# hohMiyazawa/hoh-ANS

Measured on NVIDIA B200. Metric: raw RGB MB/s, encode+decode (BASELINE.json: raw RGB MB/s encode & decode, % of HBM peak), higher is better.
Workload: dtype u8/u16 pixels, u32 freqs, u64 rANS state (integer)

## Files before the change

### hoh-ans_b200/csrc/hoh_api.cu

```cuda
#include <cuda_runtime.h>

#include <algorithm>
#include <cmath>
#include <cstdio>
#include <cstdlib>
#include <cstring>
#include <map>
#include <string>
#include <vector>

#include "hoh_kernels.cuh"

using namespace hohk;

namespace {

enum Slot {
    S_FREQS = 0, S_CUM, S_HEADS, S_ENCMETA, S_DECMETA, S_RESID, S_STREAMS, S_DSTREAMS, S_DRESULTS,
    S_IO_A, S_IO_B, S_IO_C, S_IO_D, S_IO_E, S_RESULTS, S_TOP, S_BP, S_HIST, S_COST, S_SUMS, S_MASKS,
    S_WIDE_TOP, S_WIDE_BP, S_MISC, S_L_MAPS, S_L_IDX, S_L_HDR, S_L_U32, S_L_STATUS, S_L_RR, S_L_RES, S_LZ_PX, S_LZ_STATE, S_LZ_SIDE, S_LZ_COUNTS, S_LZ_SLABS, S_LZ_RES, S_LZ_BONUS, S_LZ_KEYS, S_LZ_VALS, S_LZ_FLAG, S_T_NUKE, S_T_LZ, S_T_U32, S_T_P8, S_T_P9, S_T_O8, S_T_O9, S_T_R8, S_T_R9, S_T_MORE_SHAPES, S_T_LAST = S_T_NUKE + 4 * 9 - 1, S_D_TILES, S_D_PLANES, S_D_LZSYM, S_D_IDXSYM, S_D_RESID, S_D_OUT, S_D_BACKREF, S_D_MAPS,
    S_D_STREAMS, S_D_RES_A, S_D_RES_B, S_D_TOP, S_D_BP, S_D_PSTATUS, S_L_NEED, S_L_ORDER, S_COUNT
};

struct Buf {
// ... 772 lines not shown
    if (stream_len == 0 || stream_len % 8 || slab_bytes % 16) return HOH_E_ARG;
    if (n == 0) return HOH_OK;
    const uint64_t streams = (n + stream_len - 1) / stream_len;
    const unsigned sgrid = blocks_for(streams, kStaticWarps * 32);
    if (prob_bits >= 14) {
        k_rans_encode_static<0><<<sgrid, kStaticWarps * 32, 0, ctx->stream>>>(d_symbols, n, stream_len, d_cum, range, prob_bits, d_out,
                                                                          slab_bytes, d_payload_bytes);
    } else {
        k_rans_encode_static<1><<<sgrid, kStaticWarps * 32, 0, ctx->stream>>>(d_symbols, n, stream_len, d_cum, range, prob_bits, d_out,
                                                                          slab_bytes, d_payload_bytes);
    }
    LAUNCHED("k_rans_encode_static");
    return HOH_OK;
}

int hoh_rans_decode_static(hoh_ctx* ctx, const uint8_t* d_in, uint32_t slab_bytes,
                           const uint32_t* d_payload_bytes, size_t n, uint32_t stream_len,
                           const uint32_t* d_cum, uint32_t range, uint32_t prob_bits, uint16_t* d_symbols) {
    DeviceGuard guard_(ctx);
    if (!ctx || !d_symbols || !d_cum || !d_in || !d_payload_bytes) return HOH_E_ARG;
    if (range == 0 || range > HOH_MAX_RANGE || prob_bits == 0 || prob_bits > HOH_MAX_PROB_BITS) return HOH_E_UNSUPPORTED;
    if (stream_len == 0 || stream_len % 8 || slab_bytes % 16) return HOH_E_ARG;
    if (n == 0) return HOH_OK;
    const uint64_t streams = (n + stream_len - 1) / stream_len;
    if (prob_bits <= 15) {
        const size_t sym_bytes = range <= 256 ? 1 : 2;
        const size_t smem = (size_t)kStaticDirectWarps * 32 * kRingWords * 4 + (size_t)kStaticDirectWarps * 32 * kDecStride * 2 +
                            (size_t)HOH_MAX_RANGE * 4 + ((size_t)sym_bytes << prob_bits);
        TRY(ensure_smem_opt_in(ctx));
        const unsigned blocks = blocks_for(streams, kStaticDirectWarps * 32);
        if (range <= 256)
            k_rans_decode_static_direct<uint8_t><<<blocks, kStaticDirectWarps * 32, smem, ctx->stream>>>(
                d_in, slab_bytes, d_payload_bytes, n, stream_len, d_cum, range, prob_bits, d_symbols);
        else
            k_rans_decode_static_direct<uint16_t><<<blocks, kStaticDirectWarps * 32, smem, ctx->stream>>>(
                d_in, slab_bytes, d_payload_bytes, n, stream_len, d_cum, range, prob_bits, d_symbols);
        LAUNCHED("k_rans_decode_static_direct");
        return HOH_OK;
    }
    k_rans_decode_static<<<blocks_for(streams, kStaticDecWarps * 32), kStaticDecWarps * 32, 0, ctx->stream>>>(
        d_in, slab_bytes, d_payload_bytes, n, stream_len, d_cum, range, prob_bits, d_symbols);
    LAUNCHED("k_rans_decode_static");
    return HOH_OK;
}

int hoh_tile_geometry_for(uint32_t width, uint32_t height, hoh_tile_geometry* out) {
    if (!out || width == 0 || height == 0) return HOH_E_ARG;
    hoh_tile_geometry g;
    g.width = width;
    g.height = height;
    if ((width >= 512 || height >= 512) && width >= 256 && height >= 256) {
        g.x_tiles = width / 256;
        g.y_tiles = height / 256;
    } else {
        g.x_tiles = g.y_tiles = 1;
    }
    g.tile_w = (width + g.x_tiles - 1) / g.x_tiles;
    g.tile_h = (height + g.y_tiles - 1) / g.y_tiles;
    g.tiles_per_image = g.x_tiles * g.y_tiles;
    g.streams_per_image = 3 * g.tiles_per_image;
    *out = g;
    return HOH_OK;
}

size_t hoh_encode_images_out_bytes(const hoh_tile_geometry* g, size_t n_images) {
    if (!g) return 0;
    return hoh_enc_slab_bytes((size_t)g->tile_w * g->tile_h, 15) * g->streams_per_image * n_images;
}

int hoh_encode_images_s0(hoh_ctx* ctx, const uint8_t* d_rgb, size_t n_images, uint32_t width, uint32_t height,
                         const uint8_t* d_nuke, uint8_t* d_out, size_t out_bytes, hoh_stream_result* d_results,
                         uint8_t* d_packed, size_t packed_cap, uint64_t* d_packed_off) {
    DeviceGuard guard_(ctx);
    if (!ctx || !d_rgb || !d_out || !d_results) return HOH_E_ARG;
    if (n_images == 0) return HOH_OK;
    hoh_tile_geometry hg;
    TRY(hoh_tile_geometry_for(width, height, &hg));
    if ((uint64_t)hg.tile_w * hg.tile_h >= (1u << 21)) return HOH_E_UNSUPPORTED;
    const TileGeom g = to_geom(hg);
    const uint64_t n_tiles = (uint64_t)n_images * g.tiles_per_image, n_streams = n_tiles * 3;
    const uint32_t slab = (uint32_t)hoh_enc_slab_bytes((size_t)g.tile_w * g.tile_h, 15);
    if (out_bytes < n_streams * slab) return HOH_E_CAPACITY;
    uint16_t* resid;
    uint32_t* freqs;
    hoh_enc_stream* streams;
    TRY(scratch_t(ctx, S_RESID, n_streams * g.plane_stride, &resid));
    TRY(scratch_t(ctx, S_FREQS, n_streams * kFreqRow, &freqs));
    TRY(scratch_t(ctx, S_STREAMS, n_streams, &streams));
    if (g.width % 4 == 0 && g.tile_w % 4 == 0 && g.tile_w <= 1024) {
        k_tile_residuals_s0<<<(unsigned)n_tiles, 256, 0, ctx->stream>>>(d_rgb, g, resid, freqs);
    } else {
        k_tile_residuals_s0_generic<<<(unsigned)n_tiles, 256, 0, ctx->stream>>>(d_rgb, g, resid, freqs);
    }
    LAUNCHED("k_tile_residuals_s0");
    k_make_tile_streams<<<blocks_for(n_streams, 256), 256, 0, ctx->stream>>>(g, n_tiles, slab, streams);
    LAUNCHED("k_make_tile_streams");
    if (d_nuke) {
        k_compact_nuke<<<blocks_for(n_streams * 32, 128), 128, 0, ctx->stream>>>(g, n_tiles, d_nuke, g.plane_stride, resid,
                                                                                streams);
        LAUNCHED("k_compact_nuke");
        k_histogram<<<(unsigned)n_streams, 256, 0, ctx->stream>>>(streams, resid, freqs);
        LAUNCHED("k_histogram");
    }
    TRY(encode_from_freqs(ctx, streams, n_streams, resid, d_out, d_results, freqs, 512, 15, 15, true));
    if (d_packed) {
        if (!d_packed_off) return HOH_E_ARG;
        k_scan_sizes<<<1, 1024, 0, ctx->stream>>>(d_results, (uint32_t)n_streams, d_packed_off);
        LAUNCHED("k_scan_sizes");
        k_gather_streams<<<(unsigned)n_streams, 256, 0, ctx->stream>>>(d_results, d_out, d_packed_off, d_packed,
                                                                       packed_cap);
        LAUNCHED("k_gather_streams");
    }
    return HOH_OK;
}


int hoh_decode_images_s0(hoh_ctx* ctx, const uint8_t* d_packed, size_t packed_bytes, const uint64_t* d_packed_off,
                         size_t n_images, uint32_t width, uint32_t height, const uint16_t* d_backref,
                         uint8_t* d_rgb, int32_t* d_status) {
    DeviceGuard guard_(ctx);
    if (!ctx || !d_packed || !d_packed_off || !d_rgb || !d_status) return HOH_E_ARG;
    if (n_images == 0) return HOH_OK;
    if (packed_bytes < 32) return HOH_E_ARG;
    hoh_tile_geometry hg;
    TRY(hoh_tile_geometry_for(width, height, &hg));
    const TileGeom g = to_geom(hg);
    const uint64_t n_tiles = (uint64_t)n_images * g.tiles_per_image, n_streams = n_tiles * 3;
    uint16_t* resid;
    hoh_dec_stream* streams;
    hoh_dec_result* results;
    TRY(scratch_t(ctx, S_DSTREAMS, n_streams, &streams));
    TRY(scratch_t(ctx, S_DRESULTS, n_streams, &results));
    const bool fused = !d_backref && g.tile_w * g.x_tiles == g.width && g.tile_h * g.y_tiles == g.height && g.tile_w % 8 == 0 &&
                       g.tile_w >= 16 && g.width % 8 == 0 && (reinterpret_cast<uintptr_t>(d_rgb) & 7u) == 0 &&
                       !getenv("HOH_NO_FUSED_DECODE");
    if (fused) {
        uint32_t* cum;
        DecMeta* meta;
        TRY(scratch_t(ctx, S_CUM, n_streams * kCumRow, &cum));
        TRY(scratch_t(ctx, S_DECMETA, n_streams, &meta));
        TRY(ensure_smem_opt_in(ctx));
        k_make_tile_dec_streams<<<blocks_for(n_streams, 256), 256, 0, ctx->stream>>>(g, n_tiles, d_packed, packed_bytes,
                                                                                     d_packed_off, streams, d_status);
        LAUNCHED("k_make_tile_dec_streams");
        k_parse_streams<<<blocks_for(n_streams, kTableWarps), kTableWarps * 32, 0, ctx->stream>>>(
            streams, (uint32_t)n_streams, d_packed, packed_bytes, cum, meta, results);
        LAUNCHED("k_parse_streams");
        const uint32_t classes[5] = {0, 64, 128, 256, HOH_MAX_RANGE + 3};
        const bool overlap = !ctx->profiling;
        if (overlap) TRY(aux_fork(ctx, 4));
        const unsigned grid = blocks_for(n_tiles, kFusedTiles);
        for (int c = 0; c < 4; c++) {
            const uint32_t rows = classes[c + 1];
            const size_t fixed = (size_t)rows * 32 * sizeof(uint32_t) + 32 * kRingWords * sizeof(uint32_t) + kFusedStage;
            const size_t lut_bytes = (size_t)kLutSize * 32 * (rows <= 256 ? 1 : 2);
            const size_t smem = smem_even_share(ctx, fixed + lut_bytes, grid);
            cudaStream_t sc = overlap ? ctx->aux[c] : ctx->stream;
            if (rows <= 256) {
                k_rans_decode_tiles_s0<uint8_t><<<grid, 32, smem, sc>>>(
                    streams, (uint32_t)n_streams, d_packed, packed_bytes, cum, meta, results, g, d_rgb, d_status, classes[c], rows);
            } else {
                k_rans_decode_tiles_s0<uint16_t><<<grid, 32, smem, sc>>>(
                    streams, (uint32_t)n_streams, d_packed, packed_bytes, cum, meta, results, g, d_rgb, d_status, classes[c], rows);
            }
            static const char* const names[4] = {"k_rans_decode_tiles_s0[rows<=64]", "k_rans_decode_tiles_s0[rows<=128]",
                                                 "k_rans_decode_tiles_s0[rows<=256]", "k_rans_decode_tiles_s0[rows<=515]"};
            LAUNCHED(names[c]);
        }
        if (overlap) TRY(aux_join(ctx, 4));
        return HOH_OK;
    }
    TRY(scratch_t(ctx, S_RESID, n_streams * g.plane_stride, &resid));
    const size_t unp_smem = (size_t)kUnpWarps * ((32 * kRingStride + g.tile_w + (g.tile_w + 1) / 2 + 3) & ~(size_t)3) * sizeof(uint32_t);
    if (unp_smem > 200 * 1024) return HOH_E_UNSUPPORTED;
    k_make_tile_dec_streams<<<blocks_for(n_streams, 256), 256, 0, ctx->stream>>>(g, n_tiles, d_packed, packed_bytes,
                                                                                 d_packed_off, streams, d_status);
    LAUNCHED("k_make_tile_dec_streams");
    TRY(decode_common(ctx, streams, n_streams, d_packed, packed_bytes, resid, results));
    k_merge_status<<<blocks_for(n_streams, 256), 256, 0, ctx->stream>>>(results, n_streams, g, d_backref ? 0u : 1u, d_status);
    LAUNCHED("k_merge_status");
    if (d_backref) {
        uint16_t* planes;
        TRY(scratch_t(ctx, S_D_OUT, n_streams * g.plane_stride, &planes));
        k_tile_unpredict_s0_backref<<<blocks_for(n_streams, 64), 64, 0, ctx->stream>>>(resid, g, n_tiles, results, d_backref,
                                                                                      planes, d_status);
        LAUNCHED("k_tile_unpredict_s0_backref");
        k_tile_store_s0<<<(unsigned)n_tiles, 256, 0, ctx->stream>>>(planes, g, d_rgb);
// ... 1306 lines not shown
```

### hoh-ans_b200/csrc/hoh_kernels.cuh

```cuda
#pragma once
#include <cuda_runtime.h>
#include <stdint.h>

#include <type_traits>

#include "../../include/hohgpu.h"
#include "hoh_format.cuh"

namespace hohk {

constexpr int kFreqRow = 512;
constexpr int kCumRow = 520;
constexpr int kChunk = 64;
static_assert(true, "");
constexpr int kGroup = 8;
constexpr int kSymStride = 66;
constexpr uint64_t kRansL = 1ull << 31;
constexpr int kDecChunk = 32;
constexpr int kDecStride = 34;
constexpr uint32_t kSymBits = 9;
constexpr uint32_t kSymMask = (1u << kSymBits) - 1u;

struct EncMeta {
    uint64_t payload_start;
// ... 320 lines not shown
    }
    if (!__all_sync(0xffffffffu, fits)) {
        uint32_t len = 0;
        if (lane == 0) len = hohfmt::build_head(f, range, n, prob_bits, buf, stored_size);
        len = __shfl_sync(0xffffffffu, len, 0);
        *stored_size = __shfl_sync(0xffffffffu, *stored_size, 0);
        __syncwarp();
        return len;
    }
    const uint32_t pair_bits = mode == 2u ? 2u * count * maxbits : 0u;
    uint32_t bit = warp_incl_scan(my_bits) - my_bits + 8u * at + pair_bits;
    const uint32_t total_bits = __shfl_sync(0xffffffffu, bit + my_bits, 31);
    if (lane == 0) {
        for (uint32_t k = 0; k < at; k++) bits_or(words, 8u * k, scratch[20 + k], 8u);
        if (mode == 2u)
            for (uint32_t j = 0; j < count; j++) {
                const uint32_t c = scratch[4 + j];
                bits_or(words, 8u * at + 2u * j * maxbits, c & 0xffffu, maxbits);
                bits_or(words, 8u * at + (2u * j + 1u) * maxbits, c >> 16, maxbits);
            }
    }
    for (uint32_t i = lo; i < hi; i++) {
        uint32_t w;
        if (mode == 1u) {
            w = maxbits;
        } else {
            w = 0;
            for (uint32_t j = 0; j < count; j++) {
                const uint32_t c = scratch[4 + j];
                if ((c & 0xffffu) <= i && (c >> 16) >= i) w = j == 0 ? 1u : 4u * j;
            }
            w = min(w, prob_bits);
        }
        bits_or(words, bit, f[i], w);
        bit += w;
    }
    __syncwarp();
    const uint32_t len = (total_bits + 7u) / 8u;
    for (uint32_t k = lane; k < (len + 3u) / 4u; k += 32) words[k] = __byte_perm(words[k], 0u, 0x0123);
    __syncwarp();
    return len;
}

constexpr int kTableWarps = 4;

__device__ __forceinline__ uint32_t warp_estimate_words(const uint32_t* __restrict__ counts, const uint32_t* f,
                                                        uint32_t range, uint32_t n, uint32_t bits) {
    const uint32_t lane = lane_id();
    double S = 0.0, B = 0.0;
    uint32_t seen = 0;
    for (uint32_t i = lane; i < range; i += 32) {
        const uint32_t c = counts[i];
        if (c != 0u) {
            const double fi = (double)f[i];
            S += (double)c * ((double)bits - log2(fi));
            B += (double)c * fi;
            seen += c;
        }
    }
#pragma unroll
    for (int d = 16; d > 0; d >>= 1) {
        S += __shfl_xor_sync(0xffffffffu, S, d);
        B += __shfl_xor_sync(0xffffffffu, B, d);
        seen += __shfl_xor_sync(0xffffffffu, seen, d);
    }
    if (seen != n) return 0xff000000u;
    B *= 1.45 / 2147483648.0;
    const double k = 1.45 * exp2((double)bits - 31.0);
    const double w_cap = floor((S + B + 1.0) / 32.0) + 1.0;
    const double slack = 1e-4 + 1e-12 * S;
    const double e_hi = B + w_cap * k + slack, e_lo = -(B + 2.0 * w_cap * k + slack);
    const double lo = fmax(0.0, floor((S + e_lo) / 32.0)), hi = floor((S + e_hi) / 32.0);
    if (hi - lo > 254.0 || hi >= 16777216.0) return 0xff000000u;
    return (uint32_t)lo | ((uint32_t)(hi - lo) << 24);
}
__device__ __forceinline__ uint32_t stream_size_for(const hoh_enc_stream& st, const EncMeta& m, uint32_t words) {
    if (m.status != HOH_S_OK) return 0u;
    if (st.n == 0u) return st.prefix_len + m.head_len;
    const uint32_t payload = 4u * words + 8u;
    const uint32_t coded = m.head_len + hohfmt::varint_len(payload) + payload;
    return st.prefix_len + (m.stored_size < coded ? m.stored_size : coded);
}

__global__ void __launch_bounds__(kTableWarps * 32) k_build_tables(
    const hoh_enc_stream* __restrict__ streams, uint32_t n_streams, const uint32_t* __restrict__ freqs,
    uint32_t* __restrict__ cumtab, uint8_t* __restrict__ heads, EncMeta* __restrict__ meta) {
    __shared__ uint32_t s_f[kTableWarps][kFreqRow];
    __shared__ uint32_t s_sc[kTableWarps][kFreqRow];
    __shared__ uint32_t s_cum[kTableWarps][kFreqRow + 8];
    __shared__ __align__(16) uint8_t s_head[kTableWarps][HOH_HEAD_CAP];
    const uint32_t w = threadIdx.x >> 5, lane = lane_id();
    const uint32_t s = blockIdx.x * kTableWarps + w;
    if (s >= n_streams) return;
    const hoh_enc_stream st = streams[s];
    EncMeta m;
    m.payload_start = 0;
    m.payload_bytes = 0;
    m.head_len = 0;
    m.stored_size = 0;
    m.status = HOH_S_OK;
    m.table_u16 = st.prob_bits <= 15 ? 1u : 0u;
    m.win_lo = 0;
    m.win_rows = 0;
    m.est = 0xff000000u;
    uint8_t* head = heads + (size_t)s * HOH_HEAD_CAP;
    if (st.n == 0) {
        if (lane == 0) {
            uint32_t at = hohfmt::put_varint(s_head[w], 0, st.range - 1);
            at = hohfmt::put_varint(s_head[w], at, 0);
            for (uint32_t k = 0; k < at; k++) head[k] = s_head[w][k];
            m.head_len = at;
            meta[s] = m;
        }
        return;
    }
    uint32_t* f = s_f[w];
    uint32_t* sc = s_sc[w];
    uint32_t* cum = s_cum[w];
    const uint32_t* src = freqs + (size_t)s * kFreqRow;
    for (uint32_t i = lane; i < st.range; i += 32) f[i] = src[i];
    __syncwarp();
    int status = warp_normalize(f, sc, cum, st.range, 1u << st.prob_bits);
    if (status != HOH_S_OK) {
        if (lane == 0) {
            m.status = status;
            meta[s] = m;
        }
        return;
    }
    if ((st.reserved & HOH_FIX_LONE) && st.range > 1u) {
        uint32_t lone = 0xffffffffu;
        for (uint32_t i = lane; i < st.range; i += 32)
            if (f[i] == (1u << st.prob_bits)) lone = i;
        lone = warp_min(lone);
        if (lone != 0xffffffffu) {
            if (lane == 0) {
                f[lone] -= 1u;
                f[lone + 1u < st.range ? lone + 1u : lone - 1u] = 1u;
            }
            __syncwarp();
            warp_cumsum(f, cum, st.range);
        }
    }
    uint32_t* ct = cumtab + (size_t)s * kCumRow;
    for (uint32_t i = lane; i <= st.range; i += 32) ct[i] = cum[i];
    {
        uint32_t lo = 0xffffffffu, hi = 0u;
        for (uint32_t i = lane; i < st.range; i += 32)
            if (f[i] != 0u) {
                lo = min(lo, i);
                hi = max(hi, i);
            }
        lo = warp_min(lo);
#pragma unroll
        for (int d = 16; d > 0; d >>= 1) hi = max(hi, __shfl_xor_sync(0xffffffffu, hi, d));
        m.win_lo = lo;
        m.win_rows = hi - lo + 2u;
    }
    m.head_len = warp_build_head(f, st.range, st.n, st.prob_bits, s_head[w], sc, &m.stored_size, st.reserved & HOH_FIX_LONE);
    __syncwarp();
    m.est = warp_estimate_words(src, f, st.range, st.n, st.prob_bits);
    const uint32_t words = (m.head_len + 3u) / 4u;
    for (uint32_t k = lane; k < words; k += 32)
        reinterpret_cast<uint32_t*>(head)[k] = reinterpret_cast<const uint32_t*>(s_head[w])[k];
    if (lane == 0) meta[s] = m;
}


__device__ __forceinline__ double recip_low(uint32_t f) {
    const double fd = (double)f;
    double r;
    asm("rcp.approx.ftz.f64 %0, %1;" : "=d"(r) : "d"(fd));
    double e = fma(-fd, r, 1.0);
    r = fma(r, e, r);
    e = fma(-fd, r, 1.0);
    r = fma(r, e, r);
    return r * 0.99999999999999911182;
}

template <int DIV>
__device__ __forceinline__ uint64_t rans_put(uint64_t x, uint32_t start, uint32_t freq, double inv, uint32_t bits,
                                             uint32_t* __restrict__ words, uint32_t& widx) {
    const uint32_t xh = (uint32_t)(x >> 32), xl = (uint32_t)x;
    const bool emit = (xh >> (31u - bits)) >= freq;
    if (emit) words[--widx] = xl;
    double d_full, d_hi;
    asm("cvt.rz.f64.u64 %0, %1;" : "=d"(d_full) : "l"(x));
    asm("cvt.rn.f64.u32 %0, %1;" : "=d"(d_hi) : "r"(xh));
    const double xd = emit ? d_hi : d_full;
    x = emit ? (uint64_t)xh : x;
    uint64_t q;
    if (DIV == 1) {
        q = __double2ull_rz(xd * inv);
    } else {
        q = (uint64_t)__double_as_longlong(__fma_rz(xd, inv, 0x1p+52)) & 0x000fffffffffffffull;
    }
    uint32_t r = (uint32_t)x - (uint32_t)q * freq;
    if (r >= freq) {
        r -= freq;
        q++;
    }
    if (DIV != 0) {
        while (r >= freq) {
            r -= freq;
            q++;
        }
    }
    return (q << bits) | (uint64_t)(r + start);
}

__device__ __host__ __forceinline__ uint64_t rans_words_bound(uint64_t n, uint32_t bits) {
    return (n * bits + 32u) / 32u + 4u;
}

template <typename CumT>
struct PerLaneTable {
    const CumT* tab;
    uint32_t lane;
    __device__ __forceinline__ uint32_t cum(uint32_t s) const { return tab[s * 32u + lane]; }
};
template <typename CumT>
struct SharedTable {
    const CumT* tab;
    __device__ __forceinline__ uint32_t cum(uint32_t s) const { return tab[s]; }
};

__device__ __forceinline__ void cp_async4(uint32_t smem_addr, const void* gptr, uint32_t src_bytes) {
    asm volatile("cp.async.ca.shared.global [%0], [%1], 4, %2;" ::"r"(smem_addr), "l"(gptr), "r"(src_bytes) : "memory");
}
__device__ __forceinline__ void stage_wait() {
    asm volatile("cp.async.wait_all;" ::: "memory");
    __syncwarp();
}
template <int STRIDE = kSymStride>
__device__ __forceinline__ void stage_load_chunk(uint16_t* stage, const uint16_t* __restrict__ symbols,
                                                 const uint64_t* s_off, const uint32_t* s_n, uint32_t chunk) {
    const uint32_t lane = lane_id(), half = lane >> 4, q = lane & 15u;
    const uint32_t stage_addr = (uint32_t)__cvta_generic_to_shared(stage);
#pragma unroll 4
    for (uint32_t jj = 0; jj < 16; jj++) {
        const uint32_t r = 2u * jj + half;
        const uint32_t first = chunk * kChunk + 4u * q;
        const uint32_t n = s_n[r];
        const uint32_t left = n > first ? min(n - first, 4u) : 0u;
        const uint16_t* src = symbols + s_off[r] + (left ? first : 0u);
        const uint32_t dst = stage_addr + (r * (STRIDE / 2) + 2u * q) * 4u;
        cp_async4(dst, src, min(left, 2u) * 2u);
        cp_async4(dst + 4u, src + (left > 2u ? 2 : 0), left > 2u ? (left - 2u) * 2u : 0u);
// ... 1931 lines not shown
    uint32_t plane_stride;
};

__device__ __forceinline__ void tile_rect(const TileGeom& g, uint32_t tile, uint32_t& x0, uint32_t& y0,
                                          uint32_t& tw, uint32_t& th) {
    x0 = (tile % g.x_tiles) * g.tile_w;
    y0 = (tile / g.x_tiles) * g.tile_h;
    tw = min(g.tile_w, g.width - x0);
    th = min(g.tile_h, g.height - y0);
}

struct TileSel {
    TileGeom g;
    uint32_t x_first, x_count, y_first, y_count, per_image;
};

__device__ __forceinline__ void sel_tile(const TileSel& s, uint64_t lt, uint64_t& image, uint32_t& tile_in_image,
                                         uint32_t& x0, uint32_t& y0, uint32_t& tw, uint32_t& th) {
    image = lt / s.per_image;
    const uint32_t k = (uint32_t)(lt % s.per_image);
    const uint32_t tx = s.x_first + k % s.x_count, ty = s.y_first + k / s.x_count;
    tile_in_image = ty * s.g.x_tiles + tx;
    tile_rect(s.g, tile_in_image, x0, y0, tw, th);
}

__global__ void __launch_bounds__(256) k_tile_residuals_s0_generic(const uint8_t* __restrict__ rgb, TileGeom g,
                                                           uint16_t* __restrict__ resid,
                                                           uint32_t* __restrict__ freqs) {
    __shared__ uint32_t s_h[3][kFreqRow];
    for (int i = threadIdx.x; i < 3 * kFreqRow; i += blockDim.x) (&s_h[0][0])[i] = 0;
    __syncthreads();
    const uint64_t t = blockIdx.x;
    const uint64_t image = t / g.tiles_per_image;
    const uint32_t tile = (uint32_t)(t % g.tiles_per_image);
    uint32_t x0, y0, tw, th;
    tile_rect(g, tile, x0, y0, tw, th);
    const uint8_t* img = rgb + image * (uint64_t)g.width * g.height * 3u;
    uint16_t* out_g = resid + (t * 3u + 0u) * g.plane_stride;
    uint16_t* out_rg = resid + (t * 3u + 1u) * g.plane_stride;
    uint16_t* out_bg = resid + (t * 3u + 2u) * g.plane_stride;
    const uint32_t px = tw * th;
    for (uint32_t i = threadIdx.x; i < px; i += blockDim.x) {
        const uint32_t x = i % tw, y = i / tw;
        const uint8_t* p = img + ((uint64_t)(y0 + y) * g.width + x0 + x) * 3u;
        const int64_t up = -(int64_t)g.width * 3;
        const int r = p[0], gg = p[1], b = p[2];
        int Lg = 128, Lr = 256, Lb = 256, Tg = 128, Tr = 256, Tb = 256, TLg = 128, TLr = 256, TLb = 256;
        if (x) {
            const int lr = p[-3], lg = p[-2], lb = p[-1];
            Lg = lg;
            Lr = lr - lg + 256;
            Lb = lb - lg + 256;
        }
        if (y) {
            const int tr = p[up], tg = p[up + 1], tb = p[up + 2];
            Tg = tg;
            Tr = tr - tg + 256;
            Tb = tb - tg + 256;
            if (x) {
                const int ar = p[up - 3], ag = p[up - 2], ab = p[up - 1];
                TLg = ag;
                TLr = ar - ag + 256;
                TLb = ab - ag + 256;
            }
        }
        const int vg = gg, vr = r - gg + 256, vb = b - gg + 256;
        const int rg_ = (vg - p_med_grad(Tg, Lg, TLg) + 128 + 256) & 255;
        const int rr_ = (vr - p_med_grad(Tr, Lr, TLr) + 256 + 512) & 511;
        const int rb_ = (vb - p_med_grad(Tb, Lb, TLb) + 256 + 512) & 511;
        out_g[i] = (uint16_t)rg_;
        out_rg[i] = (uint16_t)rr_;
        out_bg[i] = (uint16_t)rb_;
        atomicAdd(&s_h[0][rg_], 1u);
        atomicAdd(&s_h[1][rr_], 1u);
        atomicAdd(&s_h[2][rb_], 1u);
    }
    __syncthreads();
    for (int ch = 0; ch < 3; ch++) {
        uint32_t* dst = freqs + (t * 3u + ch) * kFreqRow;
        for (int i = threadIdx.x; i < kFreqRow; i += blockDim.x) dst[i] = s_h[ch][i];
    }
}

__global__ void __launch_bounds__(256) k_tile_residuals_s0(const uint8_t* __restrict__ rgb, TileGeom g,
                                                           uint16_t* __restrict__ resid,
                                                           uint32_t* __restrict__ freqs) {
    __shared__ uint32_t s_h[3][kFreqRow];
    for (int i = threadIdx.x; i < 3 * kFreqRow; i += blockDim.x) (&s_h[0][0])[i] = 0;
    __syncthreads();
    const uint64_t t = blockIdx.x;
    const uint64_t image = t / g.tiles_per_image;
    const uint32_t tile = (uint32_t)(t % g.tiles_per_image);
    uint32_t x0, y0, tw, th;
    tile_rect(g, tile, x0, y0, tw, th);
    const uint8_t* img = rgb + image * (uint64_t)g.width * g.height * 3u;
    uint16_t* out_g = resid + (t * 3u + 0u) * g.plane_stride;
    uint16_t* out_rg = resid + (t * 3u + 1u) * g.plane_stride;
    uint16_t* out_bg = resid + (t * 3u + 2u) * g.plane_stride;
    const uint32_t quads = tw / 4u;
    const uint32_t qpt = min(quads, 256u);
    const uint32_t n_bands = 256u / qpt, band_rows = (th + n_bands - 1u) / n_bands;
    const uint32_t band = threadIdx.x / qpt;
    const uint32_t row_words = g.width * 3u / 4u;
    if (band < n_bands) {
        const uint32_t ya = band * band_rows, yb = min(th, ya + band_rows);
        for (uint32_t q = threadIdx.x % qpt; q < quads && ya < yb; q += qpt) {
            const uint32_t* row = reinterpret_cast<const uint32_t*>(img + ((uint64_t)(y0 + ya) * g.width + x0 + 4u * q) * 3u);
            uint32_t tg[5], tr[5];
            if (ya) {
                const uint32_t* up = row - row_words;
                const uint32_t u0 = up[0], u1 = up[1], u2 = up[2];
                planes2_of(u0 & 0xffffffu, tg[1], tr[1]);
                planes2_of((u0 >> 24) | ((u1 & 0xffffu) << 8), tg[2], tr[2]);
                planes2_of((u1 >> 16) | ((u2 & 0xffu) << 16), tg[3], tr[3]);
                planes2_of(u2 >> 8, tg[4], tr[4]);
                if (q) planes2_of(up[-1] >> 8, tg[0], tr[0]);
            } else {
#pragma unroll
                for (int i = 1; i < 5; i++) {
                    tg[i] = 128u;
                    tr[i] = kHalfRB;
                }
            }
            if (!q || !ya) {
                tg[0] = 128u;
                tr[0] = kHalfRB;
            }
            uint32_t n0 = row[0], n1 = row[1], n2 = row[2], nl = q ? row[-1] : 0u;
            uint32_t at = ya * tw + 4u * q;
            for (uint32_t y = ya; y < yb; y++, at += tw) {
                const uint32_t w0 = n0, w1 = n1, w2 = n2, wl = nl;
                if (y + 1u < yb) {
                    row += row_words;
                    n0 = row[0];
                    n1 = row[1];
                    n2 = row[2];
                    if (q) nl = row[-1];
                }
                uint32_t cg[5], cr[5];
                planes2_of(w0 & 0xffffffu, cg[1], cr[1]);
                planes2_of((w0 >> 24) | ((w1 & 0xffffu) << 8), cg[2], cr[2]);
                planes2_of((w1 >> 16) | ((w2 & 0xffu) << 16), cg[3], cr[3]);
                planes2_of(w2 >> 8, cg[4], cr[4]);
                if (q) {
                    planes2_of(wl >> 8, cg[0], cr[0]);
                } else {
                    cg[0] = 128u;
                    cr[0] = kHalfRB;
                }
                uint32_t rg_[4], rr_[4];
#pragma unroll
                for (int i = 0; i < 4; i++) {
                    rg_[i] = (cg[i + 1] - p_med_grad2(tg[i + 1], cg[i], tg[i]) + 128u + 256u) & 255u;
                    rr_[i] = __vadd2(__vsub2(cr[i + 1], p_med_grad2(tr[i + 1], cr[i], tr[i])), kHalfRB) & kMaskRB;
                    atomicAdd(&s_h[0][rg_[i]], 1u);
                    atomicAdd(&s_h[1][rr_[i] & 0xffffu], 1u);
                    atomicAdd(&s_h[2][rr_[i] >> 16], 1u);
                }
                *reinterpret_cast<uint2*>(out_g + at) = make_uint2(rg_[0] | (rg_[1] << 16), rg_[2] | (rg_[3] << 16));
                *reinterpret_cast<uint2*>(out_rg + at) =
                    make_uint2(__byte_perm(rr_[0], rr_[1], 0x5410), __byte_perm(rr_[2], rr_[3], 0x5410));
                *reinterpret_cast<uint2*>(out_bg + at) =
                    make_uint2(__byte_perm(rr_[0], rr_[1], 0x7632), __byte_perm(rr_[2], rr_[3], 0x7632));
#pragma unroll
                for (int i = 0; i < 5; i++) {
                    tg[i] = cg[i];
                    tr[i] = cr[i];
                }
            }
        }
    }
    __syncthreads();
    for (int ch = 0; ch < 3; ch++) {
        uint32_t* dst = freqs + (t * 3u + ch) * kFreqRow;
        for (int i = threadIdx.x; i < kFreqRow; i += blockDim.x) dst[i] = s_h[ch][i];
    }
}

__global__ void k_make_tile_streams(TileGeom g, uint64_t n_tiles, uint32_t slab_bytes,
                                    hoh_enc_stream* __restrict__ streams) {
    const uint64_t s = blockIdx.x * (uint64_t)blockDim.x + threadIdx.x;
    if (s >= n_tiles * 3u) return;
    const uint64_t t = s / 3u;
    const uint32_t ch = (uint32_t)(s % 3u);
    uint32_t x0, y0, tw, th;
    tile_rect(g, (uint32_t)(t % g.tiles_per_image), x0, y0, tw, th);
    hoh_enc_stream st;
    st.sym_off = s * g.plane_stride;
    st.n = tw * th;
    st.range = ch == 0 ? 256u : 512u;
    st.prob_bits = 15;
    st.prefix_len = 5;
    st.prefix[0] = 0x10;
    st.prefix[1] = 0;
    st.prefix[2] = 0;
    st.prefix[3] = 0x00;
    st.prefix[4] = 0x10;
    st.prefix[5] = st.prefix[6] = st.prefix[7] = 0;
    st.out_off = s * (uint64_t)slab_bytes;
    st.out_cap = slab_bytes;
    st.reserved = 0;
    streams[s] = st;
}

__global__ void k_make_tile_dec_streams(TileGeom g, uint64_t n_tiles, const uint8_t* __restrict__ packed,
                                        uint64_t packed_bytes, const uint64_t* __restrict__ packed_off,
                                        hoh_dec_stream* __restrict__ streams, int32_t* __restrict__ status) {
    const uint64_t s = blockIdx.x * (uint64_t)blockDim.x + threadIdx.x;
    if (s >= n_tiles * 3u) return;
    const uint64_t off = packed_off[s];
    const ByteView b{packed, packed_bytes};
    const bool ok = b[off] == 0x10 && b[off + 1] == 0 && b[off + 2] == 0 && b[off + 3] == 0 && b[off + 4] == 0x10;
    uint32_t x0, y0, tw, th;
    tile_rect(g, (uint32_t)((s / 3u) % g.tiles_per_image), x0, y0, tw, th);
    hoh_dec_stream st;
    st.in_off = off + 5u;
    st.sym_off = s * g.plane_stride;
    st.sym_cap = ok ? tw * th : 0u;
    st.flags = HOH_FIX_ALL;
    streams[s] = st;
    status[s] = ok ? HOH_S_OK : HOH_S_BAD_LAYER;
}

constexpr int kRingStride = 66;
constexpr int kUnpWarps = 4;
constexpr int kUnpBlock = 16;
constexpr uint32_t kMidPacked = 128u | (256u << 8) | (256u << 17);

struct UnpPrefetch {
    uint2 g[4], a[4], b[4];
};
template <bool ALIGNED>
__device__ __forceinline__ void unp_fetch_block(UnpPrefetch& pf, const uint16_t* __restrict__ in_g,
                                                const uint16_t* __restrict__ in_rg,
                                                const uint16_t* __restrict__ in_bg, uint32_t y_base, uint32_t th,
                                                uint32_t tw, uint32_t block) {
    const uint32_t lane = lane_id();
    const uint32_t c = kUnpBlock * block + 4u * (lane & 3u);
#pragma unroll
    for (uint32_t i = 0; i < 4; i++) {
        const uint32_t y = y_base + 8u * i + (lane >> 2);
        pf.g[i] = pf.a[i] = pf.b[i] = make_uint2(0u, 0u);
        if (y < th && c < tw) {
            const uint32_t at = y * tw + c;
            if (ALIGNED) {
                pf.g[i] = *reinterpret_cast<const uint2*>(in_g + at);
                pf.a[i] = *reinterpret_cast<const uint2*>(in_rg + at);
                pf.b[i] = *reinterpret_cast<const uint2*>(in_bg + at);
            } else {
                uint32_t v[3][4];
#pragma unroll
                for (uint32_t k = 0; k < 4; k++) {
                    const bool ok = c + k < tw;
                    v[0][k] = ok ? in_g[at + k] : 0u;
                    v[1][k] = ok ? in_rg[at + k] : 0u;
                    v[2][k] = ok ? in_bg[at + k] : 0u;
                }
                pf.g[i] = make_uint2(v[0][0] | (v[0][1] << 16), v[0][2] | (v[0][3] << 16));
// ... 2132 lines not shown
```

Before: 265,800.

## Fuse tile residual histogramming with per-stream table building in a warp-specialized persistent kernel

Adds a persistent kernel in which six warps compute tile residuals and histograms into double-buffered shared memory while three warps normalize frequencies and build the cumulative tables, headers and metadata for the previous tile. Named barriers coordinate the producer and consumer warps. This removes the global round trip of the frequency rows and the separate table-building launch on the common no-nuke quad path. The cost is fewer pixel threads per tile, occupancy limits from the added shared memory, and barrier coordination overhead.

Result: no change. 266,100 (median of 6 runs) (+0.1%).

```diff
diff --git a/hoh-ans_b200/csrc/hoh_api.cu b/hoh-ans_b200/csrc/hoh_api.cu
--- a/hoh-ans_b200/csrc/hoh_api.cu
+++ b/hoh-ans_b200/csrc/hoh_api.cu
@@ -878,27 +878,45 @@
     const uint32_t slab = (uint32_t)hoh_enc_slab_bytes((size_t)g.tile_w * g.tile_h, 15);
     if (out_bytes < n_streams * slab) return HOH_E_CAPACITY;
     uint16_t* resid;
-    uint32_t* freqs;
     hoh_enc_stream* streams;
     TRY(scratch_t(ctx, S_RESID, n_streams * g.plane_stride, &resid));
-    TRY(scratch_t(ctx, S_FREQS, n_streams * kFreqRow, &freqs));
     TRY(scratch_t(ctx, S_STREAMS, n_streams, &streams));
-    if (g.width % 4 == 0 && g.tile_w % 4 == 0 && g.tile_w <= 1024) {
-        k_tile_residuals_s0<<<(unsigned)n_tiles, 256, 0, ctx->stream>>>(d_rgb, g, resid, freqs);
-    } else {
-        k_tile_residuals_s0_generic<<<(unsigned)n_tiles, 256, 0, ctx->stream>>>(d_rgb, g, resid, freqs);
-    }
-    LAUNCHED("k_tile_residuals_s0");
     k_make_tile_streams<<<blocks_for(n_streams, 256), 256, 0, ctx->stream>>>(g, n_tiles, slab, streams);
     LAUNCHED("k_make_tile_streams");
-    if (d_nuke) {
-        k_compact_nuke<<<blocks_for(n_streams * 32, 128), 128, 0, ctx->stream>>>(g, n_tiles, d_nuke, g.plane_stride, resid,
-                                                                                streams);
-        LAUNCHED("k_compact_nuke");
-        k_histogram<<<(unsigned)n_streams, 256, 0, ctx->stream>>>(streams, resid, freqs);
-        LAUNCHED("k_histogram");
-    }
-    TRY(encode_from_freqs(ctx, streams, n_streams, resid, d_out, d_results, freqs, 512, 15, 15, true));
+    const bool quads = g.width % 4 == 0 && g.tile_w % 4 == 0 && g.tile_w <= 1024;
+    if (quads && !d_nuke) {
+        uint32_t* cum;
+        uint8_t* heads;
+        EncMeta* meta;
+        TRY(scratch_t(ctx, S_CUM, n_streams * kCumRow, &cum));
+        TRY(scratch_t(ctx, S_HEADS, n_streams * HOH_HEAD_CAP, &heads));
+        TRY(scratch_t(ctx, S_ENCMETA, n_streams, &meta));
+        int per_sm = 0;
+        CK(cudaOccupancyMaxActiveBlocksPerMultiprocessor(&per_sm, k_tile_residuals_tables_s0, kResidTablesThreads, 0));
+        const uint64_t ctas = std::min<uint64_t>(n_tiles, (uint64_t)std::max(per_sm, 1) * (uint64_t)ctx->sm_count);
+        k_tile_residuals_tables_s0<<<(unsigned)ctas, kResidTablesThreads, 0, ctx->stream>>>(d_rgb, g, n_tiles, resid,
+                                                                                          streams, cum, heads, meta);
+        LAUNCHED("k_tile_residuals_tables_s0");
+        TRY(ensure_smem_opt_in(ctx));
+        TRY(encode_with_tables(ctx, streams, n_streams, resid, d_out, d_results, cum, heads, meta, 512, 15, 15, true));
+    } else {
+        uint32_t* freqs;
+        TRY(scratch_t(ctx, S_FREQS, n_streams * kFreqRow, &freqs));
+        if (quads) {
+            k_tile_residuals_s0<<<(unsigned)n_tiles, 256, 0, ctx->stream>>>(d_rgb, g, resid, freqs);
+        } else {
+            k_tile_residuals_s0_generic<<<(unsigned)n_tiles, 256, 0, ctx->stream>>>(d_rgb, g, resid, freqs);
+        }
+        LAUNCHED("k_tile_residuals_s0");
+        if (d_nuke) {
+            k_compact_nuke<<<blocks_for(n_streams * 32, 128), 128, 0, ctx->stream>>>(g, n_tiles, d_nuke, g.plane_stride,
+                                                                                    resid, streams);
+            LAUNCHED("k_compact_nuke");
+            k_histogram<<<(unsigned)n_streams, 256, 0, ctx->stream>>>(streams, resid, freqs);
+            LAUNCHED("k_histogram");
+        }
+        TRY(encode_from_freqs(ctx, streams, n_streams, resid, d_out, d_results, freqs, 512, 15, 15, true));
+    }
     if (d_packed) {
         if (!d_packed_off) return HOH_E_ARG;
         k_scan_sizes<<<1, 1024, 0, ctx->stream>>>(d_results, (uint32_t)n_streams, d_packed_off);
diff --git a/hoh-ans_b200/csrc/hoh_kernels.cuh b/hoh-ans_b200/csrc/hoh_kernels.cuh
--- a/hoh-ans_b200/csrc/hoh_kernels.cuh
+++ b/hoh-ans_b200/csrc/hoh_kernels.cuh
@@ -426,17 +426,19 @@
     return st.prefix_len + (m.stored_size < coded ? m.stored_size : coded);
 }
 
-__global__ void __launch_bounds__(kTableWarps * 32) k_build_tables(
-    const hoh_enc_stream* __restrict__ streams, uint32_t n_streams, const uint32_t* __restrict__ freqs,
-    uint32_t* __restrict__ cumtab, uint8_t* __restrict__ heads, EncMeta* __restrict__ meta) {
-    __shared__ uint32_t s_f[kTableWarps][kFreqRow];
-    __shared__ uint32_t s_sc[kTableWarps][kFreqRow];
-    __shared__ uint32_t s_cum[kTableWarps][kFreqRow + 8];
-    __shared__ __align__(16) uint8_t s_head[kTableWarps][HOH_HEAD_CAP];
-    const uint32_t w = threadIdx.x >> 5, lane = lane_id();
-    const uint32_t s = blockIdx.x * kTableWarps + w;
-    if (s >= n_streams) return;
-    const hoh_enc_stream st = streams[s];
+struct TableScratch {
+    uint32_t f[kFreqRow];
+    uint32_t sc[kFreqRow];
+    uint32_t cum[kFreqRow + 8];
+    __align__(16) uint8_t head[HOH_HEAD_CAP];
+};
+
+__device__ __noinline__ void warp_stream_tables(const hoh_enc_stream& st, size_t s, const uint32_t* counts,
+                                                TableScratch& t, uint32_t* __restrict__ cumtab,
+                                                uint8_t* __restrict__ heads, EncMeta* __restrict__ meta) {
+    const uint32_t lane = lane_id();
+    uint32_t *f = t.f, *sc = t.sc, *cum = t.cum;
+    uint8_t* head_buf = t.head;
     EncMeta m;
     m.payload_start = 0;
     m.payload_bytes = 0;
@@ -447,22 +449,18 @@
     m.win_lo = 0;
     m.win_rows = 0;
     m.est = 0xff000000u;
-    uint8_t* head = heads + (size_t)s * HOH_HEAD_CAP;
+    uint8_t* head = heads + s * HOH_HEAD_CAP;
     if (st.n == 0) {
         if (lane == 0) {
-            uint32_t at = hohfmt::put_varint(s_head[w], 0, st.range - 1);
-            at = hohfmt::put_varint(s_head[w], at, 0);
-            for (uint32_t k = 0; k < at; k++) head[k] = s_head[w][k];
+            uint32_t at = hohfmt::put_varint(head_buf, 0, st.range - 1);
+            at = hohfmt::put_varint(head_buf, at, 0);
+            for (uint32_t k = 0; k < at; k++) head[k] = head_buf[k];
             m.head_len = at;
             meta[s] = m;
         }
         return;
     }
-    uint32_t* f = s_f[w];
-    uint32_t* sc = s_sc[w];
-    uint32_t* cum = s_cum[w];
-    const uint32_t* src = freqs + (size_t)s * kFreqRow;
-    for (uint32_t i = lane; i < st.range; i += 32) f[i] = src[i];
+    for (uint32_t i = lane; i < st.range; i += 32) f[i] = counts[i];
     __syncwarp();
     int status = warp_normalize(f, sc, cum, st.range, 1u << st.prob_bits);
     if (status != HOH_S_OK) {
@@ -486,7 +484,7 @@
             warp_cumsum(f, cum, st.range);
         }
     }
-    uint32_t* ct = cumtab + (size_t)s * kCumRow;
+    uint32_t* ct = cumtab + s * kCumRow;
     for (uint32_t i = lane; i <= st.range; i += 32) ct[i] = cum[i];
     {
         uint32_t lo = 0xffffffffu, hi = 0u;
@@ -501,13 +499,23 @@
         m.win_lo = lo;
         m.win_rows = hi - lo + 2u;
     }
-    m.head_len = warp_build_head(f, st.range, st.n, st.prob_bits, s_head[w], sc, &m.stored_size, st.reserved & HOH_FIX_LONE);
+    m.head_len = warp_build_head(f, st.range, st.n, st.prob_bits, head_buf, sc, &m.stored_size, st.reserved & HOH_FIX_LONE);
     __syncwarp();
-    m.est = warp_estimate_words(src, f, st.range, st.n, st.prob_bits);
+    m.est = warp_estimate_words(counts, f, st.range, st.n, st.prob_bits);
     const uint32_t words = (m.head_len + 3u) / 4u;
     for (uint32_t k = lane; k < words; k += 32)
-        reinterpret_cast<uint32_t*>(head)[k] = reinterpret_cast<const uint32_t*>(s_head[w])[k];
+        reinterpret_cast<uint32_t*>(head)[k] = reinterpret_cast<const uint32_t*>(head_buf)[k];
     if (lane == 0) meta[s] = m;
+}
+
+__global__ void __launch_bounds__(kTableWarps * 32) k_build_tables(
+    const hoh_enc_stream* __restrict__ streams, uint32_t n_streams, const uint32_t* __restrict__ freqs,
+    uint32_t* __restrict__ cumtab, uint8_t* __restrict__ heads, EncMeta* __restrict__ meta) {
+    __shared__ TableScratch s_tab[kTableWarps];
+    const uint32_t w = threadIdx.x >> 5;
+    const uint32_t s = blockIdx.x * kTableWarps + w;
+    if (s >= n_streams) return;
+    warp_stream_tables(streams[s], s, freqs + (size_t)s * kFreqRow, s_tab[w], cumtab, heads, meta);
 }
 
 
@@ -2605,13 +2613,9 @@
     }
 }
 
-__global__ void __launch_bounds__(256) k_tile_residuals_s0(const uint8_t* __restrict__ rgb, TileGeom g,
-                                                           uint16_t* __restrict__ resid,
-                                                           uint32_t* __restrict__ freqs) {
-    __shared__ uint32_t s_h[3][kFreqRow];
-    for (int i = threadIdx.x; i < 3 * kFreqRow; i += blockDim.x) (&s_h[0][0])[i] = 0;
-    __syncthreads();
-    const uint64_t t = blockIdx.x;
+__device__ __forceinline__ void tile_residuals_quads(const uint8_t* __restrict__ rgb, const TileGeom& g, uint64_t t,
+                                                     uint16_t* __restrict__ resid, uint32_t (*s_h)[kFreqRow], uint32_t tid,
+                                                     uint32_t nthreads) {
     const uint64_t image = t / g.tiles_per_image;
     const uint32_t tile = (uint32_t)(t % g.tiles_per_image);
     uint32_t x0, y0, tw, th;
@@ -2621,13 +2625,13 @@
     uint16_t* out_rg = resid + (t * 3u + 1u) * g.plane_stride;
     uint16_t* out_bg = resid + (t * 3u + 2u) * g.plane_stride;
     const uint32_t quads = tw / 4u;
-    const uint32_t qpt = min(quads, 256u);
-    const uint32_t n_bands = 256u / qpt, band_rows = (th + n_bands - 1u) / n_bands;
-    const uint32_t band = threadIdx.x / qpt;
+    const uint32_t qpt = min(quads, nthreads);
+    const uint32_t n_bands = nthreads / qpt, band_rows = (th + n_bands - 1u) / n_bands;
+    const uint32_t band = tid / qpt;
     const uint32_t row_words = g.width * 3u / 4u;
     if (band < n_bands) {
         const uint32_t ya = band * band_rows, yb = min(th, ya + band_rows);
-        for (uint32_t q = threadIdx.x % qpt; q < quads && ya < yb; q += qpt) {
+        for (uint32_t q = tid % qpt; q < quads && ya < yb; q += qpt) {
             const uint32_t* row = reinterpret_cast<const uint32_t*>(img + ((uint64_t)(y0 + ya) * g.width + x0 + 4u * q) * 3u);
             uint32_t tg[5], tr[5];
             if (ya) {
@@ -2693,10 +2697,61 @@
             }
         }
     }
+}
+
+__global__ void __launch_bounds__(256) k_tile_residuals_s0(const uint8_t* __restrict__ rgb, TileGeom g,
+                                                           uint16_t* __restrict__ resid, uint32_t* __restrict__ freqs) {
+    __shared__ uint32_t s_h[3][kFreqRow];
+    for (int i = threadIdx.x; i < 3 * kFreqRow; i += blockDim.x) (&s_h[0][0])[i] = 0;
+    __syncthreads();
+    const uint64_t t = blockIdx.x;
+    tile_residuals_quads(rgb, g, t, resid, s_h, threadIdx.x, 256u);
     __syncthreads();
     for (int ch = 0; ch < 3; ch++) {
         uint32_t* dst = freqs + (t * 3u + ch) * kFreqRow;
         for (int i = threadIdx.x; i < kFreqRow; i += blockDim.x) dst[i] = s_h[ch][i];
+    }
+}
+
+constexpr uint32_t kResidWarps = 6;
+constexpr uint32_t kResidTablesThreads = (kResidWarps + 3u) * 32u;
+template <int ID, int N>
+__device__ __forceinline__ void bar_sync_n() { asm volatile("bar.sync %0, %1;" ::"n"(ID), "n"(N) : "memory"); }
+template <int ID, int N>
+__device__ __forceinline__ void bar_arrive_n() { asm volatile("bar.arrive %0, %1;" ::"n"(ID), "n"(N) : "memory"); }
+
+__global__ void __launch_bounds__(kResidTablesThreads, 4) k_tile_residuals_tables_s0(
+    const uint8_t* __restrict__ rgb, TileGeom g, uint64_t n_tiles, uint16_t* __restrict__ resid,
+    const hoh_enc_stream* __restrict__ streams, uint32_t* __restrict__ cumtab, uint8_t* __restrict__ heads,
+    EncMeta* __restrict__ meta) {
+    constexpr int kAll = (int)kResidTablesThreads, kPix = (int)kResidWarps * 32;
+    __shared__ uint32_t s_h[2][3][kFreqRow];
+    __shared__ TableScratch s_tab[3];
+    const uint32_t w = threadIdx.x >> 5;
+    if (w < 3u) {
+        bar_arrive_n<1, kAll>();
+        bar_arrive_n<2, kAll>();
+        uint32_t k = 0;
+        for (uint64_t t = blockIdx.x; t < n_tiles; t += gridDim.x, k ^= 1u) {
+            if (k == 0u) bar_sync_n<3, kAll>();
+            else bar_sync_n<4, kAll>();
+            warp_stream_tables(streams[t * 3u + w], t * 3u + w, s_h[k][w], s_tab[w], cumtab, heads, meta);
+            __syncwarp();
+            if (k == 0u) bar_arrive_n<1, kAll>();
+            else bar_arrive_n<2, kAll>();
+        }
+        return;
+    }
+    const uint32_t tid = threadIdx.x - 96u;
+    uint32_t k = 0;
+    for (uint64_t t = blockIdx.x; t < n_tiles; t += gridDim.x, k ^= 1u) {
+        if (k == 0u) bar_sync_n<1, kAll>();
+        else bar_sync_n<2, kAll>();
+        for (uint32_t i = tid; i < 3u * kFreqRow; i += kPix) (&s_h[k][0][0])[i] = 0;
+        bar_sync_n<5, kPix>();
+        tile_residuals_quads(rgb, g, t, resid, s_h[k], tid, kPix);
+        if (k == 0u) bar_arrive_n<3, kAll>();
+        else bar_arrive_n<4, kAll>();
     }
 }
 
```
